# ResearchDaniel/Correlated-Photon-Mapping-for-Interactive-Global-Illumination-of-Time-Varying-Volumetric-Data

Hardware: AMD Instinct MI355X
Metric: Mphotons/s traced+binned+gathered (higher is better)
Workload: dtype f32

## Files before the change

correlated-photon-mapping-for-interactive-global-illumination-of-time-varying-volumetric-data_amd/csrc/cpm_ctx.h:

```cpp
#pragma once
#include <hip/hip_runtime.h>
#include <stdint.h>
#include <stdio.h>
#include <string.h>

#include <string>
#include <vector>

#include "cpm/cpm_ext.h"
#include "cpm_math.hip.h"

struct cpm_prof_record { const char* name; hipEvent_t a, b; };
struct cpm_prof_entry { std::string name; double total_ms = 0; long calls = 0; };

struct cpm_ctx {
    bool profiling = false;
    std::vector<cpm_prof_record> prof_pending;
    std::vector<hipEvent_t> prof_pool;
    std::vector<cpm_prof_entry> prof_entries;
    int device = 0;
    int num_cus = 256;
    size_t lds_per_block = 160 * 1024;
    std::string last_error;
    void* scratch[8] = { nullptr, nullptr, nullptr, nullptr, nullptr, nullptr, nullptr, nullptr };
    size_t scratch_bytes[8] = { 0, 0, 0, 0, 0, 0, 0, 0 };
    float* dir_hint = nullptr;
    float emit_hint_for[3] = { 0.f, 0.f, 0.f };
    bool emit_hint_valid = false;
    struct {
        unsigned long long* step_counter = nullptr;
        unsigned long long* gather_stamps = nullptr;
        int bin_fused = 1, gather_coop = 1, gather_force_voxel = 0;
        int sort_mode = 0, sort_items = 0;
        int brick_streaming = 1, select_partition = 1;
        int stream_wg_per_cu = -1;
        int fail_next_select = 0;
        int render_bits_lds = 4096;
    } dbg;
    struct cpm_trace_order* trace_order = nullptr;
    bool trace_order_measure = false;
    size_t fast_hist_words = 0;
    int fast_hist_parity = 0;
    const void* fast_last_table = nullptr;
    float fast_last_radius = 0.f;
    int photon_layout = 0;
    struct RecordBuffer { const void* base; int layout; size_t n_records; };
    std::vector<RecordBuffer> record_buffers;
    static constexpr int kTfStageSlots = 4;
    float* tf_stage = nullptr;
    float* tf_stage_dev = nullptr;
    size_t tf_stage_floats = 0;
    hipEvent_t tf_stage_done[kTfStageSlots] = { nullptr, nullptr, nullptr, nullptr };
    int tf_stage_next = 0;
};

enum {
    CPM_SCR_SORT_KEYS = 0,
    CPM_SCR_SORT_VALS = 1,
    CPM_SCR_SORT_HIST = 2,
    CPM_SCR_BIN_KEYS = 3,
    CPM_SCR_SMALL = 4,
    CPM_SCR_MISC = 5,
    CPM_SCR_FAST_BIN = 6,
    CPM_SCR_FAST_STAGE = 7
};

struct cpm_volume {
    cpm_volume_desc desc;
    void* voxels = nullptr;
    void* quads = nullptr;
    mutable bool quads_stale = false;
    size_t bytes = 0;
};

struct cpm_sequence_delta {
    struct Transition {
        void* block = nullptr;
        bool stored = false;
        uint32_t n_runs = 0;
        uint64_t payload_bytes = 0, bytes = 0;
    };
    cpm_volume_desc desc;
    int n_steps = 0, wrap = 0, refs = 1;
    uint64_t step_bytes = 0;
    std::vector<Transition> transitions;
    double dirty_fraction = 0.0, analysis_ms = 0.0;
};

struct cpm_tf {
    int width = 0;
    float* rgba = nullptr;
    float* alpha = nullptr;
};

struct cpm_trace_order {
    int n_light_samples = 0;
    uint32_t n_chunks = 0;
// ... 117 lines not shown
```

correlated-photon-mapping-for-interactive-global-illumination-of-time-varying-volumetric-data_amd/csrc/cpm_fastvolume.hip:

```cpp
#include "cpm_ctx.h"

using namespace cpm;

namespace {

#ifndef CPM_BRICK_THREADS
#define CPM_BRICK_THREADS 1024
#endif
#ifndef CPM_BRICK_WG_PER_CU
#define CPM_BRICK_WG_PER_CU 2
#endif
#ifndef CPM_COUNT_ITEMS
#define CPM_COUNT_ITEMS 4
#endif
#ifndef CPM_BRICK_PER
#define CPM_BRICK_PER 2
#endif
constexpr int kBrickThreads = CPM_BRICK_THREADS;
constexpr int kBrickPer = CPM_BRICK_PER;
constexpr int kCountItems = CPM_COUNT_ITEMS;
constexpr int kCountTile = 1024 * kCountItems;
constexpr int kScatterItems = kCountItems;
constexpr int kScatterTile = 1024 * kScatterItems;
constexpr int kMaxBricks = 8192;
// ... 52 lines not shown
        while ((1ll << (lg[0] + lg[1] + lg[2])) * box > 56 * 1024) {
            int axis = 0;
            if (lg[1] > lg[axis]) axis = 1;
            if (lg[2] > lg[axis]) axis = 2;
            if (lg[axis] <= 3) break;
            --lg[axis];
        }
#endif
    }
    auto count = [&](int a) { return (dims[a] + (1 << lg[a]) - 1) >> lg[a]; };
    while ((long long)count(0) * count(1) * count(2) > kMaxBricks) {
        int axis = 0;
        if (count(1) > count(axis)) axis = 1;
        if (count(2) > count(axis)) axis = 2;
        ++lg[axis];
    }
    L.lx = lg[0]; L.ly = lg[1]; L.lz = lg[2];
    L.nbx = count(0); L.nby = count(1); L.nbz = count(2);
    L.nb = L.nbx * L.nby * L.nbz;
    L.bvox = 1 << (lg[0] + lg[1] + lg[2]);
    L.maxc = L.mcx = L.mcy = L.mcz = 0;
    L.halo = 0;
}
__host__ void brick_shape_for(const GridDev& G, float radius, BrickLayout& L) {
    const int dims[3] = { G.dx, G.dy, G.dz };
    int mc[3];
    candidates_per_axis(G, radius, mc);
    brick_shape(dims, L, mc);
}

constexpr int kMaxCandidates = 8;
__host__ bool brick_reach(const GridDev& G, float radius, BrickLayout& L) {
    int mc[3];
    candidates_per_axis(G, radius, mc);
    L.mcx = mc[0]; L.mcy = mc[1]; L.mcz = mc[2];
    L.maxc = mc[0] > mc[1] ? (mc[0] > mc[2] ? mc[0] : mc[2]) : (mc[1] > mc[2] ? mc[1] : mc[2]);
#ifndef CPM_HALO_FROM
#define CPM_HALO_FROM 3
#endif
    L.halo = L.maxc > CPM_HALO_FROM ? 1 : 0;
    if (!(radius > 0.f) || L.maxc > kMaxCandidates) return false;
    const int lg[3] = { L.lx, L.ly, L.lz }, nbr[3] = { L.nbx, L.nby, L.nbz };
    for (int a = 0; a < 3; ++a)
        if (mc[a] > (1 << lg[a]) && nbr[a] > 1) return false;
    return true;
}
__host__ __device__ inline int halo_pitch_x(const BrickLayout& L) { return ((1 << L.lx) + L.mcx) & ~1; }
__host__ __device__ inline int tile_voxels(const BrickLayout& L) {
    return L.halo ? halo_pitch_x(L) * ((1 << L.ly) + L.mcy - 1) * ((1 << L.lz) + L.mcz - 1) : L.bvox;
}
__host__ size_t tile_bytes_for(const GridDev& G, const BrickLayout& L) { return (size_t)(G.channels == 4 ? 3 : 1) * (size_t)tile_voxels(L) * 8; }

__host__ size_t table_entries(const BrickLayout& L) { return 2 * (size_t)L.nb + 5; }

CPM_DEV bool is_sentinel(float4 a) { return a.x == kFltMax || a.y == kFltMax || a.z == kFltMax; }

CPM_DEV void axis_range(float u, float rg, int dim, int maxc, int& s, int& e) {
    s = (int)min_(max_(__builtin_ceilf(u - rg), 0.0f), (float)dim);
    e = (int)max_(min_(__builtin_floorf(u + rg), (float)(dim - 1)), -1.0f);
    e = min(e, s + maxc - 1);
}
struct Box { int sx, ex, sy, ey, sz, ez; };
CPM_DEV bool candidate_box(const GridDev& G, float4 a, float rgx, float rgy, float rgz, int mcx, int mcy, int mcz, Box& b) {
    const f3 p = { a.x, a.y, a.z };
    const f3 u = transform_(G.t2i, p);
    axis_range(u.x, rgx, G.dx, mcx, b.sx, b.ex);
    axis_range(u.y, rgy, G.dy, mcy, b.sy, b.ey);
    axis_range(u.z, rgz, G.dz, mcz, b.sz, b.ez);
    return b.sx <= b.ex && b.sy <= b.ey && b.sz <= b.ez;
}
template <typename F>
CPM_DEV void for_each_brick(const BrickLayout& L, const Box& b, F f) {
    const int bx0 = b.sx >> L.lx, by0 = b.sy >> L.ly, bz0 = b.sz >> L.lz;
    if (L.halo) {
        f((uint32_t)bx0 + (uint32_t)L.nbx * ((uint32_t)by0 + (uint32_t)L.nby * (uint32_t)bz0));
        return;
    }
    const int bx1 = b.ex >> L.lx, by1 = b.ey >> L.ly, bz1 = b.ez >> L.lz;
    for (int bz = bz0; bz <= bz1; ++bz)
        for (int by = by0; by <= by1; ++by)
            for (int bx = bx0; bx <= bx1; ++bx)
                f((uint32_t)bx + (uint32_t)L.nbx * ((uint32_t)by + (uint32_t)L.nby * (uint32_t)bz));
}

CPM_DEV float fixed_scale(float maxpow, float k) {
    const float m = maxpow * __builtin_fabsf(k) * 0.75f;
    if (!(m > 0.f) || m > kFltMax) return 1.0f;
    const int e = (int)((__float_as_uint(m) >> 23) & 0xffu) - 126;
    int sh = 30 - e;
    sh = sh > 100 ? 100 : (sh < -100 ? -100 : sh);
    return __uint_as_float((uint32_t)(sh + 127) << 23);
}
CPM_DEV unsigned long long to_fixed(float v, float S) {
    const int q = (int)(v * S);
    return (unsigned long long)(long long)q;
}

CPM_DEV void fast_scan(const uint32_t* __restrict__ counts, const BrickLayout& L, uint32_t* __restrict__ s_start,
                       uint32_t* __restrict__ table, uint32_t* s_c, uint32_t* s_i) {
    const int t = threadIdx.x, lane = t & 63, wave = t >> 6;
    const int per = (L.nb + 1023) / 1024;
    const int b0 = min(t * per, L.nb), b1 = min(b0 + per, L.nb);
    uint32_t c = 0, it = 0;
    for (int b = b0; b < b1; ++b) { const uint32_t h = counts[b]; s_start[b] = h; c += h; it += h != 0u; }
    uint32_t ci = c, ii = it;
#pragma unroll
    for (int off = 1; off < 64; off <<= 1) {
        const uint32_t oc = __shfl_up(ci, off, 64), oi = __shfl_up(ii, off, 64);
        if (lane >= off) { ci += oc; ii += oi; }
    }
    if (lane == 63) { s_c[wave] = ci; s_i[wave] = ii; }
    __syncthreads();
    uint32_t bc = 0, bi = 0, tc = 0, ti = 0;
#pragma unroll
    for (int w = 0; w < 16; ++w) { if (w < wave) { bc += s_c[w]; bi += s_i[w]; } tc += s_c[w]; ti += s_i[w]; }
    uint32_t ac = bc + ci - c, ai = bi + ii - it;
    for (int b = b0; b < b1; ++b) {
        const uint32_t h = s_start[b];
        s_start[b] = ac;
        if (table) { table[b] = ac; if (h) table[off_items(L) + ai++] = (uint32_t)b; }
        ac += h;
    }
    if (table && t == 0) { table[L.nb] = tc; table[off_meta(L) + kMetaItems] = ti; }
}

template <int CH>
__global__ __launch_bounds__(1024) void fast_count_kernel(const float* __restrict__ photons, uint32_t rec_stride, uint32_t rec_b, int n, GridDev G,
                                                          BrickLayout L, float radius, uint32_t* __restrict__ hist, uint32_t* __restrict__ acc,
                                                          uint32_t* __restrict__ run_base) {
    extern __shared__ uint32_t s_hist[];
    __shared__ float s_mp[16];
    __shared__ uint32_t s_pairs;
    const int t = threadIdx.x;
    for (int b = t; b < L.nb; b += 1024) s_hist[b] = 0u;
    if (t == 0) s_pairs = 0u;
    const float rgx = radius * G.t2i.sx + 1e-3f, rgy = radius * G.t2i.sy + 1e-3f, rgz = radius * G.t2i.sz + 1e-3f;
    const float4* __restrict__ ph = reinterpret_cast<const float4*>(photons);
    float mp = 0.f;
    float4 a[kCountItems], a2[kCountItems];
#pragma unroll
    for (int k = 0; k < kCountItems; ++k) {
        const long long i = (long long)blockIdx.x * kCountTile + k * 1024 + t;
        a[k] = make_float4(kFltMax, kFltMax, kFltMax, 0.f); a2[k] = make_float4(0.f, 0.f, 0.f, 0.f);
        if (i < n) { a[k] = ph[(size_t)rec_stride * i]; if (CH == 4) a2[k] = ph[(size_t)rec_stride * i + rec_b]; }
    }
    __syncthreads();
#pragma unroll
    for (int k = 0; k < kCountItems; ++k) {
        if (is_sentinel(a[k])) continue;
        const float p0 = __builtin_fabsf(a[k].w);
        if (p0 <= kFltMax) mp = max_(mp, p0);
        if (CH == 4) {
            const float p1 = __builtin_fabsf(a2[k].x), p2 = __builtin_fabsf(a2[k].y);
            if (p1 <= kFltMax) mp = max_(mp, p1);
            if (p2 <= kFltMax) mp = max_(mp, p2);
        }
        Box box;
        if (candidate_box(G, a[k], rgx, rgy, rgz, L.mcx, L.mcy, L.mcz, box)) for_each_brick(L, box, [&](uint32_t key) { atomicAdd(&s_hist[key], 1u); });
    }
    for (int off = 32; off > 0; off >>= 1) mp = max_(mp, __shfl_xor(mp, off, 64));
    if ((t & 63) == 0) s_mp[t >> 6] = mp;
    __syncthreads();
    uint2* __restrict__ pairs = reinterpret_cast<uint2*>(run_base) + (size_t)blockIdx.x * (size_t)pair_stride(L);
    for (int b = t; b < L.nb; b += 4 * 1024) {
        uint32_t c[4], base[4];
#pragma unroll
        for (int q = 0; q < 4; ++q) { const int bb = b + q * 1024; c[q] = bb < L.nb ? s_hist[bb] : 0u; }
#pragma unroll
        for (int q = 0; q < 4; ++q) { base[q] = 0u; if (c[q]) base[q] = atomicAdd(&hist[b + q * 1024], c[q]); }
#pragma unroll
        for (int q = 0; q < 4; ++q) if (c[q]) pairs[1u + atomicAdd(&s_pairs, 1u)] = make_uint2((uint32_t)(b + q * 1024), base[q]);
    }
    __syncthreads();
    if (t == 0) pairs[0] = make_uint2(s_pairs, 0u);
    if (t == 0) {
        float m = s_mp[0];
#pragma unroll
        for (int w = 1; w < 16; ++w) m = max_(m, s_mp[w]);
        const uint32_t mb = __float_as_uint(m);
        if (m > 0.f && __hip_atomic_load(&acc[kAccMaxPow], __ATOMIC_RELAXED, __HIP_MEMORY_SCOPE_AGENT) < mb) atomicMax(&acc[kAccMaxPow], mb);
    }
}

template <int CH>
__global__ __launch_bounds__(1024, 8) void fast_scatter_kernel(const float* __restrict__ photons, uint32_t rec_stride, uint32_t rec_b, int n, GridDev G, BrickLayout L, float radius,
                                                            const uint32_t* __restrict__ hist, const uint32_t* __restrict__ run_base,
                                                            uint32_t* __restrict__ zero_next, int zero_words,
                                                            uint32_t* __restrict__ table, float* __restrict__ sorted) {
    extern __shared__ uint32_t s_lds[];
    uint32_t* s_start = s_lds;
    uint32_t* s_pos = s_lds + L.nb;
    __shared__ uint32_t s_c[16], s_i[16];
    const int t = threadIdx.x;
    const float rgx = radius * G.t2i.sx + 1e-3f, rgy = radius * G.t2i.sy + 1e-3f, rgz = radius * G.t2i.sz + 1e-3f;
    const float4* __restrict__ ph = reinterpret_cast<const float4*>(photons);
    const int n_tiles = (int)(((long long)n + kScatterTile - 1) / kScatterTile);
    float4 a[kScatterItems], b2[kScatterItems];
    constexpr int kPairsAhead = 2;
    uint2 pr[kPairsAhead];
    uint32_t n_pairs = 0;
    auto load = [&](int tile) {
#pragma unroll
        for (int k = 0; k < kScatterItems; ++k) {
            const long long i = (long long)tile * kScatterTile + k * 1024 + t;
            a[k] = make_float4(kFltMax, kFltMax, kFltMax, 0.f); b2[k] = make_float4(0.f, 0.f, 0.f, 0.f);
            if (i < n) { a[k] = ph[(size_t)rec_stride * i]; if (CH == 4) b2[k] = ph[(size_t)rec_stride * i + rec_b]; }
        }
        n_pairs = 0;
        if (tile < n_tiles) {
            const uint2* __restrict__ pairs = reinterpret_cast<const uint2*>(run_base) + (size_t)tile * (size_t)pair_stride(L);
            n_pairs = pairs[0].x;
#pragma unroll
            for (int q = 0; q < kPairsAhead; ++q) { const uint32_t j = (uint32_t)(q * 1024 + t); pr[q] = j < n_pairs ? pairs[1u + j] : make_uint2(0u, 0u); }
        }
    };
    auto place = [&](int tile) {
        const uint2* __restrict__ pairs = reinterpret_cast<const uint2*>(run_base) + (size_t)tile * (size_t)pair_stride(L);
#pragma unroll
        for (int q = 0; q < kPairsAhead; ++q) { const uint32_t j = (uint32_t)(q * 1024 + t); if (j < n_pairs) s_pos[pr[q].x] = s_start[pr[q].x] + pr[q].y; }
        for (uint32_t j = (uint32_t)(kPairsAhead * 1024 + t); j < n_pairs; j += 1024u) { const uint2 p = pairs[1u + j]; s_pos[p.x] = s_start[p.x] + p.y; }
    };
    load(blockIdx.x);
    for (int w = blockIdx.x * 1024 + t; w < zero_words; w += gridDim.x * 1024) zero_next[w] = 0u;
    if (blockIdx.x == 0 && t == 0) {
        table[off_meta(L) + kMetaMaxPow] = hist[L.nb + kAccMaxPow];
        table[off_meta(L) + kMetaRadius] = __float_as_uint(radius);
    }
    fast_scan(hist, L, s_start, blockIdx.x == 0 ? table : nullptr, s_c, s_i);
    __syncthreads();
    for (int tile = blockIdx.x; tile < n_tiles; tile += gridDim.x) {
        if (tile != (int)blockIdx.x) load(tile);
        place(tile);
        __syncthreads();
#pragma unroll
        for (int k = 0; k < kScatterItems; ++k) {
            Box box;
            if (is_sentinel(a[k]) || !candidate_box(G, a[k], rgx, rgy, rgz, L.mcx, L.mcy, L.mcz, box)) continue;
            for_each_brick(L, box, [&](uint32_t key) {
                const size_t pos = (size_t)atomicAdd(&s_pos[key], 1u);
                if (CH == 1) {
                    typedef float v4 __attribute__((ext_vector_type(4)));
                    const v4 q = { a[k].x, a[k].y, a[k].z, a[k].w };
                    __builtin_nontemporal_store(q, reinterpret_cast<v4*>(sorted) + pos);
                } else {
                    float4* o = reinterpret_cast<float4*>(sorted) + 2 * pos;
                    o[0] = a[k];
                    o[1] = make_float4(b2[k].x, b2[k].y, 0.f, 0.f);
                }
            });
        }
        __syncthreads();
    }
}

template <int CH, int WX >
CPM_DEV void halo_record(const GridDev& G, const BrickLayout& L, float4 a, float pg, float pb, int ox, int oy, int oz, int TX, int TY,
                         float rgx, float rgy, float rgz, float r2, float inv_r2, float k, float S, long long* __restrict__ tile, int plane) {
    Box c;
    if (!candidate_box(G, a, rgx, rgy, rgz, L.mcx, L.mcy, L.mcz, c)) return;
    const float pk = __builtin_fabsf(a.w) <= kFltMax ? (a.w * k) * S : 0.f;
    const float pkg = __builtin_fabsf(pg) <= kFltMax ? (pg * k) * S : 0.f, pkb = __builtin_fabsf(pb) <= kFltMax ? (pb * k) * S : 0.f;
    float dx2[WX];
#pragma unroll
    for (int q = 0; q < WX; ++q) { const float d = fma_(G.i2t.sx, (float)(c.sx + q), G.i2t.tx) - a.x; dx2[q] = d * d; }
    for (int vz = c.sz; vz <= c.ez; ++vz) {
        const float dz = fma_(G.i2t.sz, (float)vz, G.i2t.tz) - a.z;
        for (int vy = c.sy; vy <= c.ey; ++vy) {
            const float dy = fma_(G.i2t.sy, (float)vy, G.i2t.ty) - a.y;
            if (!(fma_(dz, dz, dy * dy) <= r2)) continue;
            const int row = (c.sx - ox) + TX * ((vy - oy) + TY * (vz - oz));
#pragma unroll
            for (int q = 0; q < WX; ++q) {
                const float d2 = fma_(dz, dz, fma_(dy, dy, dx2[q]));
                if (c.sx + q > c.ex || !(d2 <= r2)) continue;
                const float w = 0.75f * (1.0f - d2 * inv_r2);
                atomicAdd(reinterpret_cast<unsigned long long*>(tile + row + q), (unsigned long long)(long long)(int)(pk * w));
                if (CH == 4) {
                    atomicAdd(reinterpret_cast<unsigned long long*>(tile + plane + row + q), (unsigned long long)(long long)(int)(pkg * w));
                    atomicAdd(reinterpret_cast<unsigned long long*>(tile + 2 * plane + row + q), (unsigned long long)(long long)(int)(pkb * w));
                }
            }
        }
    }
}

template <int MAXC, int CH>
CPM_DEV void brick_record(const GridDev& G, float4 a, float pg, float pb, int ox, int oy, int oz, int BX, int BY, int BZ, float rgx,
                          float rgy, float rgz, float r2, float inv_r2, float k, float S, long long* __restrict__ tile, int plane) {
    Box c;
    if (!candidate_box(G, a, rgx, rgy, rgz, MAXC, MAXC, MAXC, c)) return;
    const int sx = max(c.sx, ox), ex = min(c.ex, ox + BX - 1);
    const int sy = max(c.sy, oy), ey = min(c.ey, oy + BY - 1);
    const int sz = max(c.sz, oz), ez = min(c.ez, oz + BZ - 1);
    const float pk = __builtin_fabsf(a.w) <= kFltMax ? a.w * k : 0.f;
    const float pkg = __builtin_fabsf(pg) <= kFltMax ? pg * k : 0.f, pkb = __builtin_fabsf(pb) <= kFltMax ? pb * k : 0.f;
    float dxv[MAXC], dyv[MAXC], dzv[MAXC];
    bool okx[MAXC], oky[MAXC], okz[MAXC];
#pragma unroll
    for (int q = 0; q < MAXC; ++q) {
        const int vx = sx + q, vy = sy + q, vz = sz + q;
        dxv[q] = fma_(G.i2t.sx, (float)vx, G.i2t.tx) - a.x;
        dyv[q] = fma_(G.i2t.sy, (float)vy, G.i2t.ty) - a.y;
        dzv[q] = fma_(G.i2t.sz, (float)vz, G.i2t.tz) - a.z;
        okx[q] = vx <= ex; oky[q] = vy <= ey; okz[q] = vz <= ez;
    }
    const int base = (sx - ox) + BX * ((sy - oy) + BY * (sz - oz));
#pragma unroll
    for (int qz = 0; qz < MAXC; ++qz)
#pragma unroll
        for (int qy = 0; qy < MAXC; ++qy)
#pragma unroll
            for (int qx = 0; qx < MAXC; ++qx) {
                const float d2 = fma_(dzv[qz], dzv[qz], fma_(dyv[qy], dyv[qy], dxv[qx] * dxv[qx]));
                const float w = 0.75f * (1.0f - d2 * inv_r2);
                const int idx = base + qx + BX * (qy + BY * qz);
                const bool hit = okx[qx] && oky[qy] && okz[qz] && d2 <= r2;
                const unsigned long long q0 = to_fixed(pk * w, S);
                if (hit) atomicAdd(reinterpret_cast<unsigned long long*>(tile + idx), q0);
                if (CH == 4) {
                    const unsigned long long q1 = to_fixed(pkg * w, S), q2 = to_fixed(pkb * w, S);
                    if (hit) {
                        atomicAdd(reinterpret_cast<unsigned long long*>(tile + plane + idx), q1);
                        atomicAdd(reinterpret_cast<unsigned long long*>(tile + 2 * plane + idx), q2);
                    }
                }
            }
}

#ifndef CPM_BRICK_WAVES
#define CPM_BRICK_WAVES 8
#endif
constexpr int kMaxSubBricks = 512;
template <int MAXC, int CH, bool SEG>
__global__ __launch_bounds__(kBrickThreads, (CH == 4 ? 4 : CPM_BRICK_WAVES)) void fast_brick_kernel(const float* __restrict__ sorted, const uint32_t* __restrict__ table, GridDev G,
                                                                  BrickLayout L, float radius, float k, int accumulate, float* __restrict__ out,
                                                                  uint8_t* __restrict__ marks, SegTarget st) {
    extern __shared__ long long s_tile[];
    __shared__ uint32_t s_slot[SEG ? kMaxSubBricks : 1];
    __shared__ uint32_t s_base;
    __shared__ uint8_t s_flag[kMaxSubBricks];
    const int nbx4 = (G.dx + 3) >> 2, nby4 = (G.dy + 3) >> 2;
    constexpr int CH3 = CH == 4 ? 3 : 1, STRIDE = CH == 4 ? 2 : 1;
    const int t = threadIdx.x;
    const int BX = 1 << L.lx, BY = 1 << L.ly, BZ = 1 << L.lz;
    const int words = CH3 * L.bvox;
    const float rgx = radius * G.t2i.sx + 1e-3f, rgy = radius * G.t2i.sy + 1e-3f, rgz = radius * G.t2i.sz + 1e-3f;
    const float r2 = radius * radius, inv_r2 = 1.0f / r2;
    const float S = fixed_scale(__uint_as_float(table[off_meta(L) + kMetaMaxPow]), k);
    const float invS = 1.0f / S;
    const float4* __restrict__ rec = reinterpret_cast<const float4*>(sorted);
    if (!SEG && !accumulate) {
        const size_t cells = (size_t)G.dx * G.dy * G.dz;
        if (CH == 1 && (G.dx & 3) == 0) {
            for (size_t i = ((size_t)blockIdx.x * kBrickThreads + t) * 4; i < cells; i += (size_t)gridDim.x * kBrickThreads * 4) {
                const int x = (int)(i % (size_t)G.dx), y = (int)((i / (size_t)G.dx) % (size_t)G.dy), z = (int)(i / ((size_t)G.dx * G.dy));
                const uint32_t b = (uint32_t)(x >> L.lx) + (uint32_t)L.nbx * ((uint32_t)(y >> L.ly) + (uint32_t)L.nby * (uint32_t)(z >> L.lz));
                if (table[b + 1] == table[b]) {
                    *reinterpret_cast<float4*>(out + i) = make_float4(0.f, 0.f, 0.f, 0.f);
                    if (marks && ((y | z) & 3) == 0) marks[(uint32_t)(x >> 2) + (uint32_t)nbx4 * ((uint32_t)(y >> 2) + (uint32_t)nby4 * (uint32_t)(z >> 2))] = 0;
                }
            }
        } else {
            for (size_t i = (size_t)blockIdx.x * kBrickThreads + t; i < cells; i += (size_t)gridDim.x * kBrickThreads) {
                const int x = (int)(i % (size_t)G.dx), y = (int)((i / (size_t)G.dx) % (size_t)G.dy), z = (int)(i / ((size_t)G.dx * G.dy));
                const uint32_t b = (uint32_t)(x >> L.lx) + (uint32_t)L.nbx * ((uint32_t)(y >> L.ly) + (uint32_t)L.nby * (uint32_t)(z >> L.lz));
                if (table[b + 1] != table[b]) continue;
                if (CH == 1) out[i] = 0.f; else reinterpret_cast<float4*>(out)[i] = make_float4(0.f, 0.f, 0.f, 0.f);
                if (marks && ((x | y | z) & 3) == 0) marks[(uint32_t)(x >> 2) + (uint32_t)nbx4 * ((uint32_t)(y >> 2) + (uint32_t)nby4 * (uint32_t)(z >> 2))] = 0;
            }
        }
    }
    const uint32_t n_items = table[off_meta(L) + kMetaItems];
    const uint32_t* __restrict__ items = table + off_items(L);
    for (uint32_t item = blockIdx.x; item < n_items; item += gridDim.x) {
        const uint32_t b = items[item];
        const uint32_t j0 = table[b], j1 = table[b + 1];
        const int bx = (int)(b % (uint32_t)L.nbx), by = (int)((b / (uint32_t)L.nbx) % (uint32_t)L.nby), bz = (int)(b / (uint32_t)(L.nbx * L.nby));
        const int ox = bx << L.lx, oy = by << L.ly, oz = bz << L.lz;
        float4 a[kBrickPer], a2[kBrickPer], an[kBrickPer], an2[kBrickPer];
        auto fetch = [&](uint32_t first, float4* x, float4* x2) {
#pragma unroll
            for (int q = 0; q < kBrickPer; ++q) {
                const uint32_t j = first + (uint32_t)(q * kBrickThreads + t);
                x[q] = make_float4(0.f, 0.f, 0.f, 0.f); x2[q] = x[q];
                if (j < j1) { x[q] = rec[STRIDE * (size_t)j]; if (CH == 4) x2[q] = rec[2 * (size_t)j + 1]; }
            }
        };
        fetch(j0, a, a2);
        for (int w = t; w < words; w += kBrickThreads) s_tile[w] = 0ll;
        long long* my_tile = s_tile;
        const int nsub = L.bvox >> 6;
        if (marks || SEG) for (int w = t; w < nsub; w += kBrickThreads) s_flag[w] = 0;
        __syncthreads();
        for (uint32_t first = j0; first < j1; first += (uint32_t)(kBrickPer * kBrickThreads)) {
            fetch(first + (uint32_t)(kBrickPer * kBrickThreads), an, an2);
#pragma unroll
            for (int q = 0; q < kBrickPer; ++q) {
                const uint32_t j = first + (uint32_t)(q * kBrickThreads + t);
                if (j < j1) {
                    brick_record<MAXC, CH>(G, a[q], a2[q].x, a2[q].y, ox, oy, oz, BX, BY, BZ, rgx, rgy, rgz, r2, inv_r2, k, S, my_tile, L.bvox);
                }
            }
#pragma unroll
            for (int q = 0; q < kBrickPer; ++q) { a[q] = an[q]; a2[q] = an2[q]; }
        }
        __syncthreads();
        if (SEG) {
            for (int v = t; v < L.bvox; v += kBrickThreads) {
                const int lx = v & (BX - 1), ly = (v >> L.lx) & (BY - 1), lz = v >> (L.lx + L.ly);
                if (ox + lx >= G.dx || oy + ly >= G.dy || oz + lz >= G.dz) continue;
                bool nonzero = (float)s_tile[v] * invS != 0.f;
                if (CH == 4) nonzero = nonzero || (float)s_tile[L.bvox + v] * invS != 0.f || (float)s_tile[2 * L.bvox + v] * invS != 0.f;
                if (nonzero) s_flag[(lx >> 2) + (BX >> 2) * ((ly >> 2) + (BY >> 2) * (lz >> 2))] = 1;
            }
            __syncthreads();
            if (t < 64) {
                uint32_t running = 0;
                for (int w0 = 0; w0 < nsub; w0 += 64) {
                    const int w = w0 + t;
                    const bool f = w < nsub && s_flag[w] != 0;
                    const unsigned long long m = __ballot(f);
                    if (w < nsub) s_slot[w] = f ? running + (uint32_t)__popcll(m & ((1ull << t) - 1ull)) : 0xffffffffu;
                    running += (uint32_t)__popcll(m);
                }
                if (t == 0) s_base = running ? atomicAdd(&st.ctl[0], running) : 0u;
            }
            __syncthreads();
            const size_t slot_bytes = seg_slot_bytes(CH);
            for (int idx = t; idx < nsub * 64; idx += kBrickThreads) {
// ... 342 lines not shown
    G.dx = grid->dims[0]; G.dy = grid->dims[1]; G.dz = grid->dims[2]; G.channels = grid->channels;
    if (!affine_from_matrix(grid->texture_to_index, G.t2i) || !affine_from_matrix(grid->index_to_texture, G.i2t)) return 0;
    if (!(G.t2i.sx > 0.f && G.t2i.sy > 0.f && G.t2i.sz > 0.f)) return 0;
    BrickLayout L;
    brick_shape_for(G, radius, L);
    if (!brick_reach(G, radius, L)) return 0;
    return tile_bytes_for(G, L) <= (ctx ? lds_limit(ctx) : (size_t)160 * 1024 - 1024);
}

size_t cpm_fast_record_capacity(const cpm_grid_desc* grid, int n, float radius) {
    if (!cpm_gather_fast_supported(grid, radius) || n < 0) return 0;
    GridDev G;
    G.dx = grid->dims[0]; G.dy = grid->dims[1]; G.dz = grid->dims[2]; G.channels = grid->channels;
    (void)affine_from_matrix(grid->texture_to_index, G.t2i); (void)affine_from_matrix(grid->index_to_texture, G.i2t);
    BrickLayout L;
    brick_shape_for(G, radius, L);
    (void)brick_reach(G, radius, L);
    return (size_t)n * (size_t)copies_per_photon(L);
}

int cpm_bin_fast(cpm_ctx* ctx, const float* photons8, int n, const cpm_grid_desc* grid, float radius, uint32_t* brick_table,
                 float* sorted_pos_power, cpm_stream stream) {
    if (!ctx) return CPM_ERR_INVALID_ARGUMENT;
    const int described = described_layout(ctx, photons8, nullptr);
    return cpm_bin_fast_layout(ctx, photons8, described >= 0 ? described : ctx->photon_layout, n, grid, radius, brick_table, sorted_pos_power, stream);
}

int cpm_bin_fast_layout(cpm_ctx* ctx, const float* photons8, int layout, int n, const cpm_grid_desc* grid, float radius, uint32_t* brick_table,
                        float* sorted_pos_power, cpm_stream stream) {
    CPM_ENTER(ctx);
    CPM_REQUIRE(ctx, layout == CPM_PHOTONS_INTERLEAVED || layout == CPM_PHOTONS_PLANAR, "cpm_bin_fast: photon layout");
    size_t described_n = 0;
    const bool described_planar = described_layout(ctx, photons8, &described_n) == CPM_PHOTONS_PLANAR;
    CPM_REQUIRE(ctx, !(layout == CPM_PHOTONS_PLANAR && described_planar) || (size_t)(n > 0 ? n : 0) <= described_n, "cpm_bin_fast: more records than the buffer was described with");
    const uint32_t rs = layout == CPM_PHOTONS_PLANAR ? 1u : 2u,
                   rb = layout == CPM_PHOTONS_PLANAR ? (described_planar ? (uint32_t)described_n : (uint32_t)(n > 0 ? n : 0)) : 1u;
    GridDev G;
    int rc = make_grid_dev_fast(ctx, grid, G);
    if (rc) return rc;
    CPM_REQUIRE(ctx, n >= 0, "cpm_bin_fast: n < 0");
    CPM_REQUIRE(ctx, brick_table, "cpm_bin_fast: null brick_table");
    CPM_REQUIRE(ctx, n == 0 || (photons8 && sorted_pos_power), "cpm_bin_fast: null buffer");
    CPM_REQUIRE_ALIGNED16(ctx, photons8, "cpm_bin_fast");
    CPM_REQUIRE_ALIGNED16(ctx, sorted_pos_power, "cpm_bin_fast");
    hipStream_t s = (hipStream_t)stream;
    BrickLayout L;
    brick_shape_for(G, radius, L);
    if (!brick_reach(G, radius, L) || tile_bytes_for(G, L) > lds_limit(ctx))
        return set_error(ctx, CPM_ERR_UNSUPPORTED, "cpm_bin_fast", "radius beyond 3.5 voxels along some axis (or not positive): use cpm_bin + cpm_gather");
    CPM_REQUIRE(ctx, (long long)n * copies_per_photon(L) < (1ll << 32), "cpm_bin_fast: record positions are 32-bit (n * 8 must stay below 2^32)");
    static_assert(kCountTile == kScatterTile, "count and scatter launches share the tile decomposition");
    const size_t hist_words = (size_t)L.nb + kAccWords;
    const size_t tiles = n > 0 ? (size_t)div_up(n, kCountTile) : 1;
    const size_t arena = (2 * hist_words + 2 * tiles * pair_stride(L)) * 4;
    const bool had = ctx->scratch_bytes[CPM_SCR_FAST_BIN] >= arena;
    uint32_t* base = (uint32_t*)scratch(ctx, CPM_SCR_FAST_BIN, arena);
    if (!base) return CPM_ERR_OUT_OF_MEMORY;
    if (!had || ctx->fast_hist_words != hist_words) {
        CPM_HIP_CHECK(ctx, hipMemsetAsync(base, 0, 2 * hist_words * 4, s));
        ctx->fast_hist_parity = 0;
    }
    uint32_t* hist = base + (size_t)ctx->fast_hist_parity * hist_words;
    uint32_t* zero_next = base + (size_t)(ctx->fast_hist_parity ^ 1) * hist_words;
    uint32_t* acc = hist + L.nb;
    uint32_t* run_base = base + 2 * hist_words;
    ctx->fast_hist_words = 0;
    const size_t lds = (size_t)L.nb * 4;
    if (n > 0) {
        const dim3 cgrid((unsigned)tiles);
        if (G.channels == 1) {
            rc = allow_lds(ctx, fast_count_kernel<1>, lds); if (rc) return rc;
            CPM_LAUNCH(ctx, fast_count_kernel<1>, cgrid, dim3(1024), lds, s, photons8, rs, rb, n, G, L, radius, hist, acc, run_base);
        } else {
            rc = allow_lds(ctx, fast_count_kernel<4>, lds); if (rc) return rc;
            CPM_LAUNCH(ctx, fast_count_kernel<4>, cgrid, dim3(1024), lds, s, photons8, rs, rb, n, G, L, radius, hist, acc, run_base);
        }
        CPM_LAUNCH_CHECK(ctx, "fast_count_kernel");
    }
    const int stiles = n > 0 ? div_up(n, kScatterTile) : 1, smax = 2 * ctx->num_cus;
    const dim3 sgrid((unsigned)(stiles < smax ? stiles : smax));
    if (G.channels == 1) {
        rc = allow_lds(ctx, fast_scatter_kernel<1>, 2 * lds); if (rc) return rc;
        CPM_LAUNCH(ctx, fast_scatter_kernel<1>, sgrid, dim3(1024), 2 * lds, s, photons8, rs, rb, n, G, L, radius, hist, run_base, zero_next, (int)hist_words, brick_table, sorted_pos_power);
    } else {
        rc = allow_lds(ctx, fast_scatter_kernel<4>, 2 * lds); if (rc) return rc;
        CPM_LAUNCH(ctx, fast_scatter_kernel<4>, sgrid, dim3(1024), 2 * lds, s, photons8, rs, rb, n, G, L, radius, hist, run_base, zero_next, (int)hist_words, brick_table, sorted_pos_power);
    }
    CPM_LAUNCH_CHECK(ctx, "fast_scatter_kernel");
    ctx->fast_hist_parity ^= 1;
    ctx->fast_hist_words = hist_words;
    ctx->fast_last_table = brick_table;
    ctx->fast_last_radius = radius;
    return CPM_OK;
}

int cpm_photons_convert(cpm_ctx* ctx, const float* src, int src_layout, float* dst, int dst_layout, size_t n_records, cpm_stream stream) {
    CPM_ENTER(ctx);
    CPM_REQUIRE(ctx, (src_layout == CPM_PHOTONS_INTERLEAVED || src_layout == CPM_PHOTONS_PLANAR) &&
                         (dst_layout == CPM_PHOTONS_INTERLEAVED || dst_layout == CPM_PHOTONS_PLANAR), "cpm_photons_convert: layout");
    if (n_records == 0) return CPM_OK;
    CPM_REQUIRE(ctx, src && dst && src != dst, "cpm_photons_convert: null or aliased buffers");
    CPM_REQUIRE(ctx, n_records < (1ull << 31), "cpm_photons_convert: more than 2^31 records");
    CPM_REQUIRE_ALIGNED16(ctx, src, "cpm_photons_convert");
    CPM_REQUIRE_ALIGNED16(ctx, dst, "cpm_photons_convert");
    const uint32_t n = (uint32_t)n_records;
    const uint32_t ss = src_layout == CPM_PHOTONS_PLANAR ? 1u : 2u, sb = src_layout == CPM_PHOTONS_PLANAR ? n : 1u;
    const uint32_t ds = dst_layout == CPM_PHOTONS_PLANAR ? 1u : 2u, db = dst_layout == CPM_PHOTONS_PLANAR ? n : 1u;
    CPM_LAUNCH(ctx, photons_convert_kernel, dim3((unsigned)div_up((long long)n_records, 256)), dim3(256), 0, (hipStream_t)stream,
               reinterpret_cast<const float4*>(src), ss, sb, reinterpret_cast<float4*>(dst), ds, db, n_records);
    CPM_LAUNCH_CHECK(ctx, "photons_convert_kernel");
    return CPM_OK;
}

}

namespace {

int gather_fast_impl(cpm_ctx* ctx, const float* sorted_pos_power, const uint32_t* brick_table, int n, const cpm_grid_desc* grid, float radius, float scale,
                     int accumulate, float* grid_out, uint8_t* nonzero_bricks, const SegTarget* seg, cpm_stream stream) {
    GridDev G;
    int rc = make_grid_dev_fast(ctx, grid, G);
    if (rc) return rc;
    CPM_REQUIRE(ctx, n >= 0 && radius > 0.f, "cpm_gather_fast: bad size or radius");
    CPM_REQUIRE(ctx, brick_table && (grid_out || seg) && (sorted_pos_power || n == 0), "cpm_gather_fast: null buffer");
    CPM_REQUIRE_ALIGNED16(ctx, sorted_pos_power, "cpm_gather_fast");
    if (!seg && G.channels == 4) CPM_REQUIRE_ALIGNED16(ctx, grid_out, "cpm_gather_fast");
    BrickLayout L;
    brick_shape_for(G, radius, L);
    if (!brick_reach(G, radius, L))
        return set_error(ctx, CPM_ERR_UNSUPPORTED, "cpm_gather_fast", "radius beyond 3.5 voxels along some axis: use cpm_bin + cpm_gather");
    if (!seg && L.halo) CPM_REQUIRE_ALIGNED16(ctx, grid_out, "cpm_gather_fast (boxes of 4 or more candidates)");
    size_t tile_bytes = tile_bytes_for(G, L);
    if (tile_bytes > lds_limit(ctx) || (L.bvox >> 6) > kMaxSubBricks)
        return set_error(ctx, CPM_ERR_UNSUPPORTED, "cpm_gather_fast", "brick does not fit the LDS: use cpm_bin + cpm_gather");
    if (seg && L.halo && L.bvox > kSegMergeVoxels)
        return set_error(ctx, CPM_ERR_UNSUPPORTED, "cpm_gather_fast_segment", "bricks of more than 2048 voxels: gather into a grid and use cpm_bricklist_pack_grid");
    if (ctx->fast_last_table == brick_table && ctx->fast_last_radius != radius)
        return set_error(ctx, CPM_ERR_INVALID_ARGUMENT, "cpm_gather_fast", "radius differs from the one given to cpm_bin_fast for this table");
    const float k = kInv4Pi * scale;
    hipStream_t s = (hipStream_t)stream;
    const SegTarget st = seg ? *seg : SegTarget();
    const size_t resident = (size_t)CPM_BRICK_WG_PER_CU * (size_t)ctx->num_cus;
    const dim3 bgrid((unsigned)((size_t)L.nb < resident ? (size_t)L.nb : resident));
    if (L.halo) {
#ifndef CPM_BRICK_REPL
#define CPM_BRICK_REPL 4
#endif
        int repl = 1;
        while (repl * 2 <= CPM_BRICK_REPL && tile_bytes * (size_t)(repl * 2) <= lds_limit(ctx) * 9 / 20) repl *= 2;
        const size_t stage_bytes = (size_t)L.nb * tile_bytes;
        long long* stage = (long long*)scratch(ctx, CPM_SCR_FAST_STAGE, stage_bytes);
        if (!stage) return CPM_ERR_OUT_OF_MEMORY;
        const size_t lds = tile_bytes * (size_t)repl;
        const int wide = L.mcx <= 4 ? 4 : (L.mcx <= 6 ? 6 : 8);
#define CPM_HALO_LAUNCH(CH, WX)                                                                                                          \
    do {                                                                                                                                 \
        rc = allow_lds(ctx, fast_halo_kernel<CH, WX>, lds);                                                                              \
        if (rc) return rc;                                                                                                               \
        CPM_LAUNCH(ctx, (fast_halo_kernel<CH, WX>), bgrid, dim3(kBrickThreads), lds, s, sorted_pos_power, brick_table, G, L, radius, k,   \
                   stage, repl);                                                                                                         \
    } while (0)
        if (G.channels == 1) { if (wide == 4) CPM_HALO_LAUNCH(1, 4); else if (wide == 6) CPM_HALO_LAUNCH(1, 6); else CPM_HALO_LAUNCH(1, 8); }
        else { if (wide == 4) CPM_HALO_LAUNCH(4, 4); else if (wide == 6) CPM_HALO_LAUNCH(4, 6); else CPM_HALO_LAUNCH(4, 8); }
#undef CPM_HALO_LAUNCH
        CPM_LAUNCH_CHECK(ctx, "fast_halo_kernel");
        const size_t mres = (size_t)4 * (size_t)ctx->num_cus;
        const dim3 mgrid((unsigned)(seg && (size_t)L.nb > mres ? mres : (size_t)L.nb));
        if (seg) {
            if (G.channels == 1) CPM_LAUNCH(ctx, (fast_halo_merge_kernel<1, true>), mgrid, dim3(256), 0, s, stage, brick_table, G, L, k, 0, grid_out, nullptr, st);
            else CPM_LAUNCH(ctx, (fast_halo_merge_kernel<4, true>), mgrid, dim3(256), 0, s, stage, brick_table, G, L, k, 0, grid_out, nullptr, st);
        } else {
            if (G.channels == 1) CPM_LAUNCH(ctx, (fast_halo_merge_kernel<1, false>), mgrid, dim3(256), 0, s, stage, brick_table, G, L, k, accumulate, grid_out, nonzero_bricks, st);
            else CPM_LAUNCH(ctx, (fast_halo_merge_kernel<4, false>), mgrid, dim3(256), 0, s, stage, brick_table, G, L, k, accumulate, grid_out, nonzero_bricks, st);
        }
        CPM_LAUNCH_CHECK(ctx, "fast_halo_merge_kernel");
        return CPM_OK;
    }
#define CPM_BRICK_LAUNCH(MAXC, CH, SEG)                                                                                  \
    do {                                                                                                                 \
        rc = allow_lds(ctx, fast_brick_kernel<MAXC, CH, SEG>, tile_bytes);                                               \
        if (rc) return rc;                                                                                               \
        CPM_LAUNCH(ctx, (fast_brick_kernel<MAXC, CH, SEG>), bgrid, dim3(kBrickThreads), tile_bytes, s, sorted_pos_power, brick_table, G, L,  \
                   radius, k, accumulate, grid_out, nonzero_bricks, st);                                                 \
    } while (0)
    if (seg) {
        if (G.channels == 1) { if (L.maxc <= 2) CPM_BRICK_LAUNCH(2, 1, true); else CPM_BRICK_LAUNCH(3, 1, true); }
        else { if (L.maxc <= 2) CPM_BRICK_LAUNCH(2, 4, true); else CPM_BRICK_LAUNCH(3, 4, true); }
    } else if (G.channels == 1) {
        if (L.maxc <= 2) CPM_BRICK_LAUNCH(2, 1, false); else CPM_BRICK_LAUNCH(3, 1, false);
    } else {
        if (L.maxc <= 2) CPM_BRICK_LAUNCH(2, 4, false); else CPM_BRICK_LAUNCH(3, 4, false);
    }
#undef CPM_BRICK_LAUNCH
    CPM_LAUNCH_CHECK(ctx, "fast_brick_kernel");
    return CPM_OK;
}

}

extern "C" {

int cpm_gather_fast(cpm_ctx* ctx, const float* sorted_pos_power, const uint32_t* brick_table, int n, const cpm_grid_desc* grid,
                    float radius, float scale, int accumulate, float* grid_out, cpm_stream stream) {
    return cpm_gather_fast_marked(ctx, sorted_pos_power, brick_table, n, grid, radius, scale, accumulate, grid_out, nullptr, stream);
}

int cpm_gather_fast_marked(cpm_ctx* ctx, const float* sorted_pos_power, const uint32_t* brick_table, int n, const cpm_grid_desc* grid,
                           float radius, float scale, int accumulate, float* grid_out, uint8_t* nonzero_bricks, cpm_stream stream) {
    CPM_ENTER(ctx);
    CPM_REQUIRE(ctx, !(nonzero_bricks && accumulate), "cpm_gather_fast_marked: the marks describe a volume this launch wrote whole (not with accumulate)");
    CPM_REQUIRE(ctx, grid_out, "cpm_gather_fast: null buffer");
    return gather_fast_impl(ctx, sorted_pos_power, brick_table, n, grid, radius, scale, accumulate, grid_out, nonzero_bricks, nullptr, stream);
}

int cpm_gather_fast_segment(cpm_ctx* ctx, const float* sorted_pos_power, const uint32_t* brick_table, int n, const cpm_grid_desc* grid,
                            float radius, float scale, const cpm_bricklist_segment* segment, cpm_stream stream) {
    CPM_ENTER(ctx);
    CPM_REQUIRE(ctx, segment && segment->segment && segment->control && grid, "cpm_gather_fast_segment: null segment (the root, or a communicator of one rank, gathers into its grid)");
    CPM_REQUIRE(ctx, (int)segment->channels == grid->channels, "cpm_gather_fast_segment: the segment was opened for another channel count");
    const unsigned long long nb4 = (unsigned long long)((grid->dims[0] + 3) / 4) * ((grid->dims[1] + 3) / 4) * ((grid->dims[2] + 3) / 4);
    CPM_REQUIRE(ctx, grid->dims[0] >= 1 && grid->dims[1] >= 1 && grid->dims[2] >= 1 && nb4 <= segment->room, "cpm_gather_fast_segment: the segment has no room for every brick of this grid");
    SegTarget st;
    st.seg = static_cast<unsigned char*>(segment->segment);
    st.capacity = segment->capacity; st.room = segment->room; st.ticket = segment->ticket;
    st.ctl = segment->control; st.mailbox = segment->mailbox;
    return gather_fast_impl(ctx, sorted_pos_power, brick_table, n, grid, radius, scale, 0, nullptr, nullptr, &st, stream);
}

}
```

include/cpm/cpm_profile.h:

```cpp
#ifndef CPM_CPM_PROFILE_H
#define CPM_CPM_PROFILE_H
#include "cpm/cpm_ext.h"
#ifdef __cplusplus
extern "C" {
#endif
void cpm_profile_enable(cpm_ctx* ctx, int on);
void cpm_profile_reset(cpm_ctx* ctx);
int cpm_profile_collect(cpm_ctx* ctx);
const char* cpm_profile_name(const cpm_ctx* ctx, int i);
double cpm_profile_total_ms(const cpm_ctx* ctx, int i);
long cpm_profile_calls(const cpm_ctx* ctx, int i);
void cpm_debug_set_step_counter(cpm_ctx* ctx, unsigned long long* dev_counter);
void cpm_debug_set_gather_stamps(cpm_ctx* ctx, unsigned long long* dev_stamps);
void cpm_debug_force_voxel_gather(cpm_ctx* ctx, int on);
void cpm_debug_set_gather_coop(cpm_ctx* ctx, int on);
void cpm_debug_set_brick_streaming(cpm_ctx* ctx, int on);
void cpm_debug_set_select_partition(cpm_ctx* ctx, int on);
void cpm_debug_set_bin_fused(cpm_ctx* ctx, int on);
void cpm_debug_set_sort_mode(cpm_ctx* ctx, int mode);
void cpm_debug_set_sort_items(cpm_ctx* ctx, int items);
void cpm_debug_set_stream_wg_per_cu(cpm_ctx* ctx, int n);
void cpm_debug_set_render_bits_lds(cpm_ctx* ctx, int max_bytes);
void cpm_debug_fail_next_select(cpm_ctx* ctx, int on);
struct cpm_trace_order;
int cpm_debug_trace_order_read(cpm_ctx* ctx, const struct cpm_trace_order* order, uint32_t* order_out, uint32_t* cost_out);
int cpm_debug_trace_order_write(cpm_ctx* ctx, struct cpm_trace_order* order, const uint32_t* table);
int cpm_debug_pack_grid_segment(cpm_ctx* ctx, const cpm_bricklist_segment* segment, const cpm_grid_desc* grid_desc, const float* grid,
                                const uint8_t* nonzero_bricks, cpm_stream stream);
int cpm_debug_root_add_segments(cpm_ctx* ctx, const cpm_bricklist_segment* segments, int n, const cpm_grid_desc* grid_desc, float* grid,
                                uint32_t* slot_of, cpm_stream stream);
#ifdef __cplusplus
}
#endif
#endif
```

Before: 16340.

## Emit packed brick items and empty-brick bitmask from scatter for gather

The scatter kernel's scan now writes a packed uint4 record per non-empty brick (brick id, start, count, item total) plus a bitmask of empty bricks. The gather kernel reads its work item from this packed array, prefetching the next one, instead of chasing the items list and table offsets. It also tests brick emptiness with one bit instead of two table loads during the zero-fill pass. Index math in the zero-fill switches to 32-bit with power-of-two shifts. The cost is extra scratch memory, extra writes in scatter, and reliance on host-side state linking the last table to the packed buffers.

```diff
diff --git a/correlated-photon-mapping-for-interactive-global-illumination-of-time-varying-volumetric-data_amd/csrc/cpm_ctx.h b/correlated-photon-mapping-for-interactive-global-illumination-of-time-varying-volumetric-data_amd/csrc/cpm_ctx.h
--- a/correlated-photon-mapping-for-interactive-global-illumination-of-time-varying-volumetric-data_amd/csrc/cpm_ctx.h
+++ b/correlated-photon-mapping-for-interactive-global-illumination-of-time-varying-volumetric-data_amd/csrc/cpm_ctx.h
@@ -43,6 +43,9 @@
     int fast_hist_parity = 0;
     const void* fast_last_table = nullptr;
     float fast_last_radius = 0.f;
+    const void* fast_items = nullptr;
+    const void* fast_mask = nullptr;
+    uint32_t fast_items_nb = 0;
     int photon_layout = 0;
     struct RecordBuffer { const void* base; int layout; size_t n_records; };
     std::vector<RecordBuffer> record_buffers;
diff --git a/correlated-photon-mapping-for-interactive-global-illumination-of-time-varying-volumetric-data_amd/csrc/cpm_fastvolume.hip b/correlated-photon-mapping-for-interactive-global-illumination-of-time-varying-volumetric-data_amd/csrc/cpm_fastvolume.hip
--- a/correlated-photon-mapping-for-interactive-global-illumination-of-time-varying-volumetric-data_amd/csrc/cpm_fastvolume.hip
+++ b/correlated-photon-mapping-for-interactive-global-illumination-of-time-varying-volumetric-data_amd/csrc/cpm_fastvolume.hip
@@ -128,6 +128,11 @@
 __host__ size_t tile_bytes_for(const GridDev& G, const BrickLayout& L) { return (size_t)(G.channels == 4 ? 3 : 1) * (size_t)tile_voxels(L) * 8; }
 
 __host__ size_t table_entries(const BrickLayout& L) { return 2 * (size_t)L.nb + 5; }
+__host__ size_t mask_words(const BrickLayout& L) { return 2 * (((size_t)L.nb + 63) / 64); }
+__host__ size_t gather_workgroups(const cpm_ctx* ctx, const BrickLayout& L) {
+    const size_t resident = (size_t)CPM_BRICK_WG_PER_CU * (size_t)ctx->num_cus;
+    return (size_t)L.nb < resident ? (size_t)L.nb : resident;
+}
 
 CPM_DEV bool is_sentinel(float4 a) { return a.x == kFltMax || a.y == kFltMax || a.z == kFltMax; }
 
@@ -172,8 +177,8 @@
     return (unsigned long long)(long long)q;
 }
 
-CPM_DEV void fast_scan(const uint32_t* __restrict__ counts, const BrickLayout& L, uint32_t* __restrict__ s_start,
-                       uint32_t* __restrict__ table, uint32_t* s_c, uint32_t* s_i) {
+CPM_DEV uint32_t fast_scan(const uint32_t* __restrict__ counts, const BrickLayout& L, uint32_t* __restrict__ s_start,
+                           uint32_t* __restrict__ table, uint4* __restrict__ items4, uint32_t items_live, uint32_t* s_c, uint32_t* s_i) {
     const int t = threadIdx.x, lane = t & 63, wave = t >> 6;
     const int per = (L.nb + 1023) / 1024;
     const int b0 = min(t * per, L.nb), b1 = min(b0 + per, L.nb);
@@ -194,10 +199,17 @@
     for (int b = b0; b < b1; ++b) {
         const uint32_t h = s_start[b];
         s_start[b] = ac;
-        if (table) { table[b] = ac; if (h) table[off_items(L) + ai++] = (uint32_t)b; }
+        if (table) {
+            table[b] = ac;
+            if (h) { table[off_items(L) + ai] = (uint32_t)b; items4[ai] = make_uint4((uint32_t)b, ac, h, ti); ++ai; }
+        }
         ac += h;
     }
-    if (table && t == 0) { table[L.nb] = tc; table[off_meta(L) + kMetaItems] = ti; }
+    if (table) {
+        for (uint32_t j = ti + (uint32_t)t; j < items_live; j += 1024u) items4[j] = make_uint4(0u, 0u, 0u, 0u);
+        if (t == 0) { table[L.nb] = tc; table[off_meta(L) + kMetaItems] = ti; }
+    }
+    return tc;
 }
 
 template <int CH>
@@ -262,7 +274,8 @@
 __global__ __launch_bounds__(1024, 8) void fast_scatter_kernel(const float* __restrict__ photons, uint32_t rec_stride, uint32_t rec_b, int n, GridDev G, BrickLayout L, float radius,
                                                             const uint32_t* __restrict__ hist, const uint32_t* __restrict__ run_base,
                                                             uint32_t* __restrict__ zero_next, int zero_words,
-                                                            uint32_t* __restrict__ table, float* __restrict__ sorted) {
+                                                            uint32_t* __restrict__ table, uint4* __restrict__ items4, uint32_t items_live,
+                                                            uint32_t* __restrict__ empty_mask, float* __restrict__ sorted) {
     extern __shared__ uint32_t s_lds[];
     uint32_t* s_start = s_lds;
     uint32_t* s_pos = s_lds + L.nb;
@@ -302,8 +315,15 @@
         table[off_meta(L) + kMetaMaxPow] = hist[L.nb + kAccMaxPow];
         table[off_meta(L) + kMetaRadius] = __float_as_uint(radius);
     }
-    fast_scan(hist, L, s_start, blockIdx.x == 0 ? table : nullptr, s_c, s_i);
+    const uint32_t total = fast_scan(hist, L, s_start, blockIdx.x == 0 ? table : nullptr, items4, items_live, s_c, s_i);
     __syncthreads();
+    if (blockIdx.x == 0) {
+        for (int b = t; b < ((L.nb + 63) & ~63); b += 1024) {
+            const bool e = b < L.nb && s_start[b] == (b + 1 < L.nb ? s_start[b + 1] : total);
+            const unsigned long long m = __ballot(e);
+            if ((t & 63) == 0) { empty_mask[2 * (b >> 6)] = (uint32_t)m; empty_mask[2 * (b >> 6) + 1] = (uint32_t)(m >> 32); }
+        }
+    }
     for (int tile = blockIdx.x; tile < n_tiles; tile += gridDim.x) {
         if (tile != (int)blockIdx.x) load(tile);
         place(tile);
@@ -410,7 +430,8 @@
 template <int MAXC, int CH, bool SEG>
 __global__ __launch_bounds__(kBrickThreads, (CH == 4 ? 4 : CPM_BRICK_WAVES)) void fast_brick_kernel(const float* __restrict__ sorted, const uint32_t* __restrict__ table, GridDev G,
                                                                   BrickLayout L, float radius, float k, int accumulate, float* __restrict__ out,
-                                                                  uint8_t* __restrict__ marks, SegTarget st) {
+                                                                  uint8_t* __restrict__ marks, SegTarget st, const uint4* __restrict__ items4,
+                                                                  const uint32_t* __restrict__ empty_mask) {
     extern __shared__ long long s_tile[];
     __shared__ uint32_t s_slot[SEG ? kMaxSubBricks : 1];
     __shared__ uint32_t s_base;
@@ -422,35 +443,53 @@
     const int words = CH3 * L.bvox;
     const float rgx = radius * G.t2i.sx + 1e-3f, rgy = radius * G.t2i.sy + 1e-3f, rgz = radius * G.t2i.sz + 1e-3f;
     const float r2 = radius * radius, inv_r2 = 1.0f / r2;
+    const bool packed = items4 != nullptr;
+    uint4 it = make_uint4(0u, 0u, 0u, 0u);
+    if (packed) it = items4[blockIdx.x];
     const float S = fixed_scale(__uint_as_float(table[off_meta(L) + kMetaMaxPow]), k);
     const float invS = 1.0f / S;
     const float4* __restrict__ rec = reinterpret_cast<const float4*>(sorted);
     if (!SEG && !accumulate) {
-        const size_t cells = (size_t)G.dx * G.dy * G.dz;
+        const uint32_t cells = (uint32_t)G.dx * (uint32_t)G.dy * (uint32_t)G.dz;
+        const bool pow2 = (G.dx & (G.dx - 1)) == 0 && (G.dy & (G.dy - 1)) == 0;
+        const int lgx = __builtin_ctz((unsigned)G.dx), lgy = __builtin_ctz((unsigned)G.dy);
+        auto coords = [&](uint32_t i, int& x, int& y, int& z) {
+            if (pow2) { x = (int)(i & (uint32_t)(G.dx - 1)); y = (int)((i >> lgx) & (uint32_t)(G.dy - 1)); z = (int)(i >> (lgx + lgy)); }
+            else { const uint32_t r = i / (uint32_t)G.dx; x = (int)(i - r * (uint32_t)G.dx); z = (int)(r / (uint32_t)G.dy); y = (int)(r - (uint32_t)z * (uint32_t)G.dy); }
+        };
+        auto empty = [&](uint32_t b) { return packed ? ((empty_mask[b >> 5] >> (b & 31u)) & 1u) != 0u : table[b + 1] == table[b]; };
         if (CH == 1 && (G.dx & 3) == 0) {
-            for (size_t i = ((size_t)blockIdx.x * kBrickThreads + t) * 4; i < cells; i += (size_t)gridDim.x * kBrickThreads * 4) {
-                const int x = (int)(i % (size_t)G.dx), y = (int)((i / (size_t)G.dx) % (size_t)G.dy), z = (int)(i / ((size_t)G.dx * G.dy));
+            for (uint32_t i = ((uint32_t)blockIdx.x * kBrickThreads + t) * 4u; i < cells; i += (uint32_t)gridDim.x * kBrickThreads * 4u) {
+                int x, y, z;
+                coords(i, x, y, z);
                 const uint32_t b = (uint32_t)(x >> L.lx) + (uint32_t)L.nbx * ((uint32_t)(y >> L.ly) + (uint32_t)L.nby * (uint32_t)(z >> L.lz));
-                if (table[b + 1] == table[b]) {
+                if (empty(b)) {
                     *reinterpret_cast<float4*>(out + i) = make_float4(0.f, 0.f, 0.f, 0.f);
                     if (marks && ((y | z) & 3) == 0) marks[(uint32_t)(x >> 2) + (uint32_t)nbx4 * ((uint32_t)(y >> 2) + (uint32_t)nby4 * (uint32_t)(z >> 2))] = 0;
                 }
             }
         } else {
-            for (size_t i = (size_t)blockIdx.x * kBrickThreads + t; i < cells; i += (size_t)gridDim.x * kBrickThreads) {
-                const int x = (int)(i % (size_t)G.dx), y = (int)((i / (size_t)G.dx) % (size_t)G.dy), z = (int)(i / ((size_t)G.dx * G.dy));
+            for (uint32_t i = (uint32_t)blockIdx.x * kBrickThreads + t; i < cells; i += (uint32_t)gridDim.x * kBrickThreads) {
+                int x, y, z;
+                coords(i, x, y, z);
                 const uint32_t b = (uint32_t)(x >> L.lx) + (uint32_t)L.nbx * ((uint32_t)(y >> L.ly) + (uint32_t)L.nby * (uint32_t)(z >> L.lz));
-                if (table[b + 1] != table[b]) continue;
+                if (!empty(b)) continue;
                 if (CH == 1) out[i] = 0.f; else reinterpret_cast<float4*>(out)[i] = make_float4(0.f, 0.f, 0.f, 0.f);
                 if (marks && ((x | y | z) & 3) == 0) marks[(uint32_t)(x >> 2) + (uint32_t)nbx4 * ((uint32_t)(y >> 2) + (uint32_t)nby4 * (uint32_t)(z >> 2))] = 0;
             }
         }
     }
-    const uint32_t n_items = table[off_meta(L) + kMetaItems];
+    const uint32_t n_items = packed ? (it.z ? it.w : 0u) : table[off_meta(L) + kMetaItems];
     const uint32_t* __restrict__ items = table + off_items(L);
     for (uint32_t item = blockIdx.x; item < n_items; item += gridDim.x) {
-        const uint32_t b = items[item];
-        const uint32_t j0 = table[b], j1 = table[b + 1];
+        uint32_t b, j0, j1;
+        if (packed) {
+            b = it.x; j0 = it.y; j1 = it.y + it.z;
+            if (item + gridDim.x < n_items) it = items4[item + gridDim.x];
+        } else {
+            b = items[item];
+            j0 = table[b]; j1 = table[b + 1];
+        }
         const int bx = (int)(b % (uint32_t)L.nbx), by = (int)((b / (uint32_t)L.nbx) % (uint32_t)L.nby), bz = (int)(b / (uint32_t)(L.nbx * L.nby));
         const int ox = bx << L.lx, oy = by << L.ly, oz = bz << L.lz;
         float4 a[kBrickPer], a2[kBrickPer], an[kBrickPer], an2[kBrickPer];
@@ -899,8 +938,10 @@
     static_assert(kCountTile == kScatterTile, "count and scatter launches share the tile decomposition");
     const size_t hist_words = (size_t)L.nb + kAccWords;
     const size_t tiles = n > 0 ? (size_t)div_up(n, kCountTile) : 1;
-    const size_t arena = (2 * hist_words + 2 * tiles * pair_stride(L)) * 4;
+    const size_t bin_words = (2 * hist_words + 2 * tiles * pair_stride(L) + 3) & ~(size_t)3;
+    const size_t arena = (bin_words + 4 * (size_t)L.nb + mask_words(L)) * 4;
     const bool had = ctx->scratch_bytes[CPM_SCR_FAST_BIN] >= arena;
+    ctx->fast_items = nullptr;
     uint32_t* base = (uint32_t*)scratch(ctx, CPM_SCR_FAST_BIN, arena);
     if (!base) return CPM_ERR_OUT_OF_MEMORY;
     if (!had || ctx->fast_hist_words != hist_words) {
@@ -911,6 +952,9 @@
     uint32_t* zero_next = base + (size_t)(ctx->fast_hist_parity ^ 1) * hist_words;
     uint32_t* acc = hist + L.nb;
     uint32_t* run_base = base + 2 * hist_words;
+    uint4* items4 = reinterpret_cast<uint4*>(base + bin_words);
+    uint32_t* empty_mask = base + bin_words + 4 * (size_t)L.nb;
+    const uint32_t items_live = (uint32_t)gather_workgroups(ctx, L);
     ctx->fast_hist_words = 0;
     const size_t lds = (size_t)L.nb * 4;
     if (n > 0) {
@@ -928,16 +972,17 @@
     const dim3 sgrid((unsigned)(stiles < smax ? stiles : smax));
     if (G.channels == 1) {
         rc = allow_lds(ctx, fast_scatter_kernel<1>, 2 * lds); if (rc) return rc;
-        CPM_LAUNCH(ctx, fast_scatter_kernel<1>, sgrid, dim3(1024), 2 * lds, s, photons8, rs, rb, n, G, L, radius, hist, run_base, zero_next, (int)hist_words, brick_table, sorted_pos_power);
+        CPM_LAUNCH(ctx, fast_scatter_kernel<1>, sgrid, dim3(1024), 2 * lds, s, photons8, rs, rb, n, G, L, radius, hist, run_base, zero_next, (int)hist_words, brick_table, items4, items_live, empty_mask, sorted_pos_power);
     } else {
         rc = allow_lds(ctx, fast_scatter_kernel<4>, 2 * lds); if (rc) return rc;
-        CPM_LAUNCH(ctx, fast_scatter_kernel<4>, sgrid, dim3(1024), 2 * lds, s, photons8, rs, rb, n, G, L, radius, hist, run_base, zero_next, (int)hist_words, brick_table, sorted_pos_power);
+        CPM_LAUNCH(ctx, fast_scatter_kernel<4>, sgrid, dim3(1024), 2 * lds, s, photons8, rs, rb, n, G, L, radius, hist, run_base, zero_next, (int)hist_words, brick_table, items4, items_live, empty_mask, sorted_pos_power);
     }
     CPM_LAUNCH_CHECK(ctx, "fast_scatter_kernel");
     ctx->fast_hist_parity ^= 1;
     ctx->fast_hist_words = hist_words;
     ctx->fast_last_table = brick_table;
     ctx->fast_last_radius = radius;
+    ctx->fast_items = items4; ctx->fast_mask = empty_mask; ctx->fast_items_nb = (uint32_t)L.nb;
     return CPM_OK;
 }
 
@@ -987,8 +1032,10 @@
     const float k = kInv4Pi * scale;
     hipStream_t s = (hipStream_t)stream;
     const SegTarget st = seg ? *seg : SegTarget();
-    const size_t resident = (size_t)CPM_BRICK_WG_PER_CU * (size_t)ctx->num_cus;
-    const dim3 bgrid((unsigned)((size_t)L.nb < resident ? (size_t)L.nb : resident));
+    const bool packed = ctx->fast_last_table == brick_table && ctx->fast_items && ctx->fast_items_nb == (uint32_t)L.nb;
+    const uint4* items4 = packed ? static_cast<const uint4*>(ctx->fast_items) : nullptr;
+    const uint32_t* empty_mask = packed ? static_cast<const uint32_t*>(ctx->fast_mask) : nullptr;
+    const dim3 bgrid((unsigned)gather_workgroups(ctx, L));
     if (L.halo) {
 #ifndef CPM_BRICK_REPL
 #define CPM_BRICK_REPL 4
@@ -1028,7 +1075,7 @@
         rc = allow_lds(ctx, fast_brick_kernel<MAXC, CH, SEG>, tile_bytes);                                               \
         if (rc) return rc;                                                                                               \
         CPM_LAUNCH(ctx, (fast_brick_kernel<MAXC, CH, SEG>), bgrid, dim3(kBrickThreads), tile_bytes, s, sorted_pos_power, brick_table, G, L,  \
-                   radius, k, accumulate, grid_out, nonzero_bricks, st);                                                 \
+                   radius, k, accumulate, grid_out, nonzero_bricks, st, items4, empty_mask);                             \
     } while (0)
     if (seg) {
         if (G.channels == 1) { if (L.maxc <= 2) CPM_BRICK_LAUNCH(2, 1, true); else CPM_BRICK_LAUNCH(3, 1, true); }
@@ -1058,6 +1105,18 @@
     CPM_REQUIRE(ctx, !(nonzero_bricks && accumulate), "cpm_gather_fast_marked: the marks describe a volume this launch wrote whole (not with accumulate)");
     CPM_REQUIRE(ctx, grid_out, "cpm_gather_fast: null buffer");
     return gather_fast_impl(ctx, sorted_pos_power, brick_table, n, grid, radius, scale, accumulate, grid_out, nonzero_bricks, nullptr, stream);
+}
+
+int cpm_debug_fast_items(cpm_ctx* ctx, const uint32_t* brick_table, uint32_t* items_out, uint32_t* empty_mask_out, uint32_t* n_bricks_out) {
+    CPM_ENTER(ctx);
+    CPM_REQUIRE(ctx, n_bricks_out, "cpm_debug_fast_items: null n_bricks_out");
+    const bool held = brick_table && ctx->fast_last_table == brick_table && ctx->fast_items;
+    *n_bricks_out = held ? ctx->fast_items_nb : 0u;
+    if (!held) return CPM_OK;
+    CPM_HIP_CHECK(ctx, hipDeviceSynchronize());
+    if (items_out) CPM_HIP_CHECK(ctx, hipMemcpy(items_out, ctx->fast_items, (size_t)ctx->fast_items_nb * 16, hipMemcpyDeviceToHost));
+    if (empty_mask_out) CPM_HIP_CHECK(ctx, hipMemcpy(empty_mask_out, ctx->fast_mask, 2 * (((size_t)ctx->fast_items_nb + 63) / 64) * 4, hipMemcpyDeviceToHost));
+    return CPM_OK;
 }
 
 int cpm_gather_fast_segment(cpm_ctx* ctx, const float* sorted_pos_power, const uint32_t* brick_table, int n, const cpm_grid_desc* grid,
diff --git a/include/cpm/cpm_profile.h b/include/cpm/cpm_profile.h
--- a/include/cpm/cpm_profile.h
+++ b/include/cpm/cpm_profile.h
@@ -29,6 +29,7 @@
                                 const uint8_t* nonzero_bricks, cpm_stream stream);
 int cpm_debug_root_add_segments(cpm_ctx* ctx, const cpm_bricklist_segment* segments, int n, const cpm_grid_desc* grid_desc, float* grid,
                                 uint32_t* slot_of, cpm_stream stream);
+int cpm_debug_fast_items(cpm_ctx* ctx, const uint32_t* brick_table, uint32_t* items_out, uint32_t* empty_mask_out, uint32_t* n_bricks_out);
 #ifdef __cplusplus
 }
 #endif
```

Measured after the change: 16420 (median of 6 runs). About the same (+0.5%).
